# MpokiAbel/UPMEM--OpenFHE

Hardware: AMD Instinct MI355X
Metric: 64-bit coeffs/sec for NTT+Hadamard+INTT, N=2^16, 16 towers; % HBM roofline (higher is better)
Workload: dtype u64; 1 GPU; configs[2]: N=2^16, towers=16, batch=1024 per GPU, c = INTT(NTT(a) (.) b); log_n=16, towers=16, batch_per_gpu=1024, global_batch=1024, parallelism=batch-sharded x1 (no data-path collective)

## Files before the change

upmem--openfhe_amd/csrc/arith.hpp:

```cpp
#pragma once
#include <hip/hip_runtime.h>
#include <stdint.h>

namespace ofhe {

typedef uint64_t u64;
typedef uint32_t u32;

struct VgprFloor {
    __device__ __forceinline__ ~VgprFloor() { asm volatile("" ::: "v63"); }
};
#define OFHE_VGPR_FLOOR() const VgprFloor ofhe_vgpr_floor_guard_

__device__ __forceinline__ u32 lo32(u64 x) { return (u32)x; }
__device__ __forceinline__ u32 hi32(u64 x) { return (u32)(x >> 32); }
__device__ __forceinline__ u64 pack(u32 lo, u32 hi) { return ((u64)hi << 32) | lo; }

__device__ __forceinline__ u64 mad32(u32 a, u32 b, u64 c) { return (u64)a * (u64)b + c; }

__device__ __forceinline__ u64 csub(u64 x, u64 m) { return x >= m ? x - m : x; }

__device__ __noinline__ u64 umod64(u64 v, u64 m) { return v % m; }
struct SwMod {
    u64 half, nm, diff;
// ... 51 lines not shown
    }
    if (OFHE_QH_ADDC) {
        const u32 h1 = __umulhi(lo32(a), hi32(b));
        const u32 h2 = __umulhi(hi32(a), lo32(b));
        const u32 s = h1 + h2;
        return mad32(hi32(a), hi32(b), pack(s, s < h1));
    }
    const u64 m1 = mad32(lo32(a), hi32(b), 0);
    const u64 m2 = mad32(hi32(a), lo32(b), 0);
    if (OFHE_QH_MAD1) return mad32(hi32(m2), one, mad32(hi32(a), hi32(b), m1 >> 32));
    return mad32(hi32(a), hi32(b), (m1 >> 32) + (m2 >> 32));
}

__device__ __forceinline__ u64 mulhi_exact(u64 a, u64 b) {
    u64 p00 = mad32(lo32(a), lo32(b), 0);
    u64 m1 = mad32(lo32(a), hi32(b), (u64)hi32(p00));
    u64 m2 = mad32(hi32(a), lo32(b), (u64)lo32(m1));
    u64 h = mad32(hi32(a), hi32(b), (u64)hi32(m1));
    return h + (u64)hi32(m2);
}

template <bool SPQ, bool QA = false>
struct Mod {
    u64 q;
    u64 q4;
    u64 q8;
    u64 nq;
    u64 nq4;
    u64 nq8;
    u32 sh;
    u32 one = 1;
};

template <bool SPQ, bool QA>
__device__ __forceinline__ u64 shoup_lazy(u64 a, u64 w, u64 wp, const Mod<SPQ, QA>& M) {
    const u64 qh = mulhi_approx<QA>(a, wp, M.one);
    u64 s = mad32(lo32(a), lo32(w), 0);
    s = mad32(lo32(qh), lo32(M.nq), s);
    u32 hi;
    if (SPQ)
        hi = hi32(s) + lo32(a) * hi32(w) + hi32(a) * lo32(w) - (lo32(qh) << M.sh) + hi32(qh) * lo32(M.nq);
    else
        hi = hi32(s) + lo32(a) * hi32(w) + hi32(a) * lo32(w) + lo32(qh) * hi32(M.nq) + hi32(qh) * lo32(M.nq);
    return pack(lo32(s), hi);
}

// ... 120 lines not shown
```

upmem--openfhe_amd/csrc/bconv_cols.hpp:

```cpp
#pragma once
#include "bconv_mma.hpp"

namespace ofhe {

#ifndef OFHE_BCC_STAGE_BAR
#define OFHE_BCC_STAGE_BAR 1
#endif
#ifndef OFHE_BCC_MINW
#define OFHE_BCC_MINW 3
#endif
#ifndef OFHE_BCC_WAVES
#define OFHE_BCC_WAVES 12
#endif
constexpr u32 BC_WAVES = OFHE_BCC_WAVES;
constexpr u32 BC_THREADS = 64 * BC_WAVES;
constexpr u32 BC_COLS = 16, BC_ROWS = 32, BC_POS = BC_COLS * BC_ROWS;

template <bool SPQ>
__device__ __forceinline__ void bcc_icol_source(const PlanArgs& P, const BmSrc* srcc, const u64* __restrict__ xb,
                                                u32 src, u32 src_rel, u32 lane, u64* dg64) {
    constexpr u32 N = 1u << 17, COLS = N / BC_ROWS;
    const u32 col = lane & 15, qq = lane >> 4;
    const u32 ts = src_rel + src;
    const auto M = load_mod<SPQ, (bool)OFHE_QA_CI>(P.tc[ts]);
// ... 102 lines not shown
            u64 d[2];
#pragma unroll
            for (int u = 0; u < 2; u++) {
                const u32 i = 2 * pr + u;
                u64 y = 0;
                if (i < A.size_q) {
                    const BmSrc S = srcc[i];
                    y = shoup_canon(xr[k][u], S.w, S.wp, S.q);
                }
                d[u] = digits8(y);
            }
            dg[it] = i32x4{(int)lo32(d[0]), (int)hi32(d[0]), (int)lo32(d[1]), (int)hi32(d[1])};
        }
    }
    __syncthreads();
    const BmW W = bm_weights();
    const u32 c = lane & 31, h = lane >> 5, col = c & 15, par = c >> 4;
    u64* ob = out + (u64)b * A.out_stride + c0 + col;
    auto colpass = [&](u64(&vv)[16], u32 j) {
        if (j >= A.size_p) return;
        const u32 jo = j >= A.gap_at ? j + A.gap : j;
        const auto M = load_mod<SPQ, (bool)OFHE_QA_BCC>(P.tc[jo]);
        const u64* tw = P.tw + (u64)jo * N * 2;
#pragma unroll
        for (int s = 0; s < 4; s++) {
            const int hg = 8 >> s;
#pragma unroll
            for (int jb = 0; jb < (1 << s); jb++) {
                const Tw tw_ = ldtw(tw, (1u << s) + jb);
#pragma unroll
                for (int g = jb * 2 * hg; g < jb * 2 * hg + hg; g++) ct_bfly_cs(vv[g], vv[g + hg], tw_, M, (s & 1) == 0);
            }
            if (OFHE_BCC_STAGE_BAR) __builtin_amdgcn_sched_barrier(0);
        }
        u64* oj = ob + (u64)jo * N;
#pragma unroll
        for (int k = 0; k < 8; k++) {
            const u64 snd = par ? vv[k] : vv[8 + k];
            const u64 rcv = pack((u32)__shfl_xor((int)lo32(snd), 16), (u32)__shfl_xor((int)hi32(snd), 16));
            u64 xv = par ? rcv : vv[k];
            u64 yv = par ? vv[8 + k] : rcv;
            const u32 g = k + 8 * par;
            ct_bfly_cs(xv, yv, ldtw(tw, 16 + g), M, true);
            st_s(oj + (u64)(2 * g) * COLS, xv);
            st_s(oj + (u64)(2 * g + 1) * COLS, yv);
        }
    };
#pragma unroll 1
    for (u32 T = w; T < tiles; T += BC_WAVES) {
        i32x4 fa[KS];
#pragma unroll
        for (int s = 0; s < KS; s++) fa[s] = frag[(T * KS + s) * 64 + lane];
        const BmRed R0 = red[4 * T + 2 * h], R1 = red[4 * T + 2 * h + 1];
        u64 v0[16], v1[16];
        auto mma = [&](int g) {
            i32x16 acc = {};
#pragma unroll
            for (int s = 0; s < KS; s++)
                acc = __builtin_amdgcn_mfma_i32_32x32x32_i8(fa[s], dg[(2 * s + h) * BC_POS + 32 * g + c], acc, 0, 0,
                                                             0);
            return acc;
        };
        i32x16 accn = mma(0);
#pragma unroll
        for (int g = 0; g < 16; g++) {
            const i32x16 acc = accn;
// ... 19 lines not shown
```

upmem--openfhe_amd/csrc/ntt_kernels.hpp:

```cpp
#pragma once
#include "arith.hpp"

namespace ofhe {

struct TowerConst {
    u64 q;
    u64 ninv;
    u64 ninv_pre;
    u64 mu;
    u64 nq;
    u64 nq4;
    u32 nshift;
    u32 spq_sh;
    u64 qinv;
    u32 one;
    u32 pad_;
};
#ifndef OFHE_QA_TCF
#define OFHE_QA_TCF 0
#endif
#ifndef OFHE_QA_TCI
#define OFHE_QA_TCI 0
#endif
#ifndef OFHE_QA_BLK
// ... 86 lines not shown
#define OFHE_FOLD 1
#endif
#ifndef OFHE_BFLY_ACC
#define OFHE_BFLY_ACC 1
#endif
template <bool SPQ, bool QA>
__device__ __forceinline__ u64 red16(u64 x, const Mod<SPQ, QA>& M) {
    if (SPQ && OFHE_FOLD) return fold_spq(x, M);
    return csub_s(x, M.q8);
}
#ifndef OFHE_FOLD_GS
#define OFHE_FOLD_GS 0
#endif
template <bool SPQ, bool QA>
__device__ __forceinline__ u64 red8(u64 x, const Mod<SPQ, QA>& M) {
    if (SPQ && OFHE_FOLD && OFHE_FOLD_GS) return fold_spq(x, M);
    return csub_s(x, M.q4);
}
template <bool SPQ, bool QA>
__device__ __forceinline__ u64 red16_gs(u64 x, const Mod<SPQ, QA>& M) {
    if (SPQ && OFHE_FOLD && OFHE_FOLD_GS) return fold_spq(x, M);
    return csub_s(x, M.q8);
}
template <bool SPQ, bool QA>
__device__ __forceinline__ void ct_bfly_cs(u64& x, u64& y, Tw w, const Mod<SPQ, QA>& M, bool cs) {
    u64 a;
    if (OFHE_LAZY_FWD)
        a = cs ? ((SPQ && OFHE_THR) ? csub_thr8(x, M) : red16(x, M)) : x;
    else
        a = csub_s(x, M.q4);
    if (OFHE_BFLY_ACC == 2) {
        const u64 c2 = (a << 1) + M.q4;
        x = shoup_lazy_acc(y, w.w, w.wp, M, a);
        y = c2 - x;
    } else if (OFHE_BFLY_ACC) {
        x = shoup_lazy_acc(y, w.w, w.wp, M, a);
        y = (a << 1) + M.q4 - x;
    } else {
        const u64 t = shoup_lazy(y, w.w, w.wp, M);
        x = a + t;
        y = a + M.q4 - t;
    }
}
template <int CS, class M_>
__device__ __forceinline__ void ct_bfly(u64& x, u64& y, Tw w, const M_& M) {
    ct_bfly_cs(x, y, w, M, CS != 0);
// ... 41 lines not shown
    if (SPQ && OFHE_THR) x = csub_s(x, 8 * q);
    if (OFHE_LAZY_FWD) x = csub_s(x, 8 * q);
    return canon8(x, q);
}

static_assert(OFHE_LAZY_FWD, "the DIT inverse uses the alternating lazy CT butterflies");

__device__ __forceinline__ void triv_bfly(u64& x, u64& y, u64 bq) {
    const u64 s = x + y;
    y = x + bq - y;
    x = s;
}

template <int H, int CS, class M_>
__device__ __forceinline__ void dit_stage16(u64 (&v)[16], const u64* base, u32 st, const M_& M) {
    constexpr int half = 1 << H;
#pragma unroll
    for (int j = 0; j < half; j++) {
        const Tw w = ldtw(base, st * j);
#pragma unroll
        for (int g = 0; g < 16; g += 2 * half) ct_bfly<CS>(v[g + j], v[g + j + half], w, M);
    }
}
template <class M_>
__device__ __forceinline__ void dit_round16(u64 (&v)[16], const u64* dtw, u32 st, u32 r, const M_& M) {
    dit_stage16<0, 1>(v, dtw + 2 * ((u64)st + r), st, M);
    dit_stage16<1, 0>(v, dtw + 2 * ((u64)2 * st + r), st, M);
    dit_stage16<2, 1>(v, dtw + 2 * ((u64)4 * st + r), st, M);
    dit_stage16<3, 0>(v, dtw + 2 * ((u64)8 * st + r), st, M);
}

template <bool SPQ, bool QA>
__device__ __forceinline__ void dit_round3(u64 (&v)[16], const u64* dtw, const Mod<SPQ, QA>& M) {
#pragma unroll
    for (int g = 0; g < 16; g += 2) triv_bfly(v[g], v[g + 1], 2 * M.q);
#pragma unroll
    for (int g = 0; g < 16; g += 4) triv_bfly(v[g], v[g + 2], M.q4);
    {
        const Tw w = ldtw(dtw, 3);
#pragma unroll
        for (int g = 0; g < 16; g += 4) ct_bfly<0>(v[g + 1], v[g + 3], w, M);
    }
#pragma unroll
    for (int g = 0; g < 16; g += 8) triv_bfly(v[g], v[g + 4], M.q8);
#pragma unroll
    for (int j = 1; j < 4; j++) {
        const Tw w = ldtw(dtw, 4 + j);
#pragma unroll
        for (int g = 0; g < 16; g += 8) ct_bfly<0>(v[g + j], v[g + j + 4], w, M);
    }
    {
        const u64 a = red16(v[0], M), b = red16(v[8], M);
        v[0] = a;
        v[8] = b;
        triv_bfly(v[0], v[8], M.q8);
    }
#pragma unroll
    for (int j = 1; j < 8; j++) ct_bfly<1>(v[j], v[j + 8], ldtw(dtw, 8 + j), M);
}

template <bool SPQ, bool QA>
__device__ __forceinline__ u64 twist_out(u64 x, Tw f, const Mod<SPQ, QA>& M) {
    return canon4m(shoup_lazy(x, f.w, f.wp, M), M);
}

template <int S, class M_, int CS = S & 1>
__device__ __forceinline__ void fwd_stage16(u64 (&v)[16], const u64* tw, u32 M0, const M_& M) {
    constexpr int half = 8 >> S;
    const u64* base = tw + 2 * ((u64)M0 << S);
#pragma unroll
    for (int j = 0; j < (1 << S); j++) {
        Tw w = ldtw(base, j);
#pragma unroll
        for (int k = j * 2 * half; k < j * 2 * half + half; k++) ct_bfly<CS>(v[k], v[k + half], w, M);
    }
}

template <int S, class M_>
__device__ __forceinline__ void inv_stage16(u64 (&v)[16], const u64* itw, u32 M0, const M_& M) {
    constexpr int half = 8 >> S;
    const u64* base = itw + 2 * ((u64)M0 << S);
#pragma unroll
    for (int j = 0; j < (1 << S); j++) {
        Tw w = ldtw(base, j);
#pragma unroll
        for (int k = j * 2 * half; k < j * 2 * half + half; k++) gs_bfly(v[k], v[k + half], w, M);
    }
}

#ifndef OFHE_LAZY_GS
#define OFHE_LAZY_GS 1
#endif
template <class M_>
__device__ __forceinline__ void gs_bfly_b(u64& x, u64& y, Tw w, const M_& M, bool in8) {
    const u64 s = x + y;
    const u64 d = x + (in8 ? M.q8 : M.q4) - y;
    x = in8 ? red16_gs(s, M) : s;
    y = shoup_lazy(d, w.w, w.wp, M);
}
template <int S, class M_>
__device__ __forceinline__ void inv_stage16_b(u64 (&v)[16], bool (&b8)[16], const u64* itw, u32 M0, const M_& M) {
    constexpr int half = 8 >> S;
    const u64* base = itw + 2 * ((u64)M0 << S);
#pragma unroll
    for (int j = 0; j < (1 << S); j++) {
        Tw w = ldtw(base, j);
#pragma unroll
        for (int k = j * 2 * half; k < j * 2 * half + half; k++) {
            gs_bfly_b(v[k], v[k + half], w, M, b8[k] || b8[k + half]);
            b8[k] = true;
            b8[k + half] = false;
        }
    }
}
template <class M_>
__device__ __forceinline__ void inv_round16_b(u64 (&v)[16], bool (&b8)[16], const u64* itw, u32 M0, const M_& M) {
    inv_stage16_b<3>(v, b8, itw, M0, M);
    inv_stage16_b<2>(v, b8, itw, M0, M);
    inv_stage16_b<1>(v, b8, itw, M0, M);
    inv_stage16_b<0>(v, b8, itw, M0, M);
}

template <class M_>
__device__ __forceinline__ void fwd_round16(u64 (&v)[16], const u64* tw, u32 M0, const M_& M) {
    fwd_stage16<0>(v, tw, M0, M);
    fwd_stage16<1>(v, tw, M0, M);
    fwd_stage16<2>(v, tw, M0, M);
    fwd_stage16<3>(v, tw, M0, M);
}
#ifndef OFHE_FWD_CANON
#define OFHE_FWD_CANON 1
#endif
template <class M_>
__device__ __forceinline__ void fwd_round16_canon(u64 (&v)[16], const u64* tw, u32 M0, const M_& M) {
    fwd_stage16<0>(v, tw, M0, M);
    fwd_stage16<1, M_, OFHE_FWD_CANON ? 0 : 1>(v, tw, M0, M);
    fwd_stage16<2>(v, tw, M0, M);
    fwd_stage16<3>(v, tw, M0, M);
}
template <class M_>
__device__ __forceinline__ void inv_round16(u64 (&v)[16], const u64* itw, u32 M0, const M_& M) {
    inv_stage16<3>(v, itw, M0, M);
    inv_stage16<2>(v, itw, M0, M);
    inv_stage16<1>(v, itw, M0, M);
    inv_stage16<0>(v, itw, M0, M);
}

#ifndef OFHE_TW3
#define OFHE_TW3 1
#endif
#ifndef OFHE_MONT
#define OFHE_MONT 1
#endif
#ifndef OFHE_COAL
#define OFHE_COAL 1
#endif
#ifndef OFHE_COAL_B
#define OFHE_COAL_B 1
#endif
constexpr bool kMontFused = OFHE_MONT && OFHE_COAL_B;
static_assert(!(kMontFused && OFHE_THR), "Montgomery Hadamard needs the forward output < 12q");
template <int S, class M_>
__device__ __forceinline__ void fwd_stage16_t3(u64 (&v)[16], const u64* tw3, u32 U, u32 u, const M_& M) {
    constexpr int half = 8 >> S;
    const u64* base = tw3 + 2 * (u64)(((1u << S) - 1) * U);
#pragma unroll
    for (int j = 0; j < (1 << S); j++) {
        Tw w = ldtw(base + 2 * (u64)j * U, u);
#pragma unroll
        for (int k = j * 2 * half; k < j * 2 * half + half; k++) ct_bfly<S & 1>(v[k], v[k + half], w, M);
    }
}
__device__ __forceinline__ u32 lds_pad(u32 p) { return p + (p >> 4); }
constexpr u32 LDS_WORDS = 4096 + 4096 / 16;

__device__ __forceinline__ void wave_stage_in(const u64* wsrc, u64* lds, u32 tid, u64 (&out)[16]) {
    const u32 lane = tid & 63, base = (tid >> 6) * 1024;
#pragma unroll
    for (int k = 0; k < 8; k++) {
        const u64x2 v = ld2_s(wsrc + 128 * k + 2 * lane);
        const u32 p = base + 128 * k + 2 * lane;
        lds[lds_pad(p)] = v.x;
        lds[lds_pad(p) + 1] = v.y;
    }
    __builtin_amdgcn_wave_barrier();
#pragma unroll
    for (int k = 0; k < 16; k++) out[k] = lds[tid * 17 + k];
    __builtin_amdgcn_wave_barrier();
}
template <int NPRE>
__device__ __forceinline__ void wave_stage_in_pre(const u64* wsrc, u64* lds, u32 tid, const u64x2 (&pre)[NPRE > 0 ? NPRE : 1],
                                                  u64 (&out)[16]) {
    const u32 lane = tid & 63, base = (tid >> 6) * 1024;
// ... 34 lines not shown
__device__ __forceinline__ void block_body(const PlanArgs& P, const u64* src, u64* dst, const u64* __restrict__ bdat,
                                           u32 batch, u32 wid, u64* lds, u32 tid) {
    static_assert(NR == 2 || NR == 3, "k_block covers the last 8 (NR=2) or 12 (NR=3) stages");
    static_assert(SK == 0 || (SK == 3 && NR == 3), "k_block: SK = 3 needs NR = 3");
    const u32 logn = P.log_n;
    const u32 N = 1u << logn;
    const u32 G = N >> 12;
    const u32 g = wid % G;
    const u32 pb = wid / G;
    const u32 t = pb / batch, b = pb % batch;
    const u64 inner = (u64)t * N + ((u64)g << 12);
    const u64 off = (u64)b * P.dstride + inner;
    const u64 boff = (u64)b * P.bstride + inner;
    const u64* blk = src + (u64)b * P.sstride + inner;
    u64* oblk = dst + off;
    const TowerConst tc = P.tc[t];
    const u64 q = tc.q;
    const auto M = load_mod<SPQ, (bool)OFHE_QA_BLK>(tc);
    const u64* tw = P.tw + (u64)t * N * 2;
    const u32 h = tid >> 4, r = tid & 15;
    const u32 L1 = tid + h;
    const u32 L2 = h * 272 + r;
    const u32 L3 = tid * 17;
    u64 v[16];

    if (MODE == MODE_FWD || MODE == MODE_FUSED || MODE == MODE_FWD_SUB) {
        if (NR == 3) {
#pragma unroll
            for (int k = 0; k < 16; k++) v[k] = ld_s(blk + tid + 256 * k);
            if (SK == 3)
                fwd_stage16<3>(v, tw, (N >> 12) + g, M);
            else
                fwd_round16(v, tw, (N >> 12) + g, M);
#pragma unroll
            for (int k = 0; k < 16; k++) lds[L1 + 272 * k] = v[k];
            __syncthreads();
#pragma unroll
            for (int k = 0; k < 16; k++) v[k] = lds[L2 + 17 * k];
        } else {
#pragma unroll
            for (int k = 0; k < 16; k++) v[k] = ld_s(blk + h * 256 + r + 16 * k);
        }
        fwd_round16(v, tw, (N >> 8) + g * 16 + h, M);
#pragma unroll
        for (int k = 0; k < 16; k++) lds[L2 + 17 * k] = v[k];
        __syncthreads();
#pragma unroll
        for (int k = 0; k < 16; k++) v[k] = lds[L3 + k];
        constexpr int BPF = ((MODE == MODE_FUSED && OFHE_COAL_B) || MODE == MODE_FWD_SUB) ? OFHE_B_PF : 0;
        u64x2 bpre[BPF > 0 ? BPF : 1];
#pragma unroll
        for (int k = 0; k < BPF; k++) bpre[k] = ld2_s(bdat + boff + (tid >> 6) * 1024 + 128 * k + 2 * (tid & 63));
        if (OFHE_TW3) {
            const u64* tw3 = P.tw3 + (u64)t * (N / 16) * 30;
            const u32 U = N >> 4, u = g * 256 + tid;
            fwd_stage16_t3<0>(v, tw3, U, u, M);
            fwd_stage16_t3<1>(v, tw3, U, u, M);
            fwd_stage16_t3<2>(v, tw3, U, u, M);
            fwd_stage16_t3<3>(v, tw3, U, u, M);
        } else {
            fwd_round16(v, tw, (N >> 4) + g * 256 + tid, M);
        }
        if (!(MODE == MODE_FUSED && kMontFused) && MODE != MODE_FWD_SUB) {
#pragma unroll
            for (int k = 0; k < 16; k++) v[k] = canon_fwd<SPQ>(v[k], M);
        }
        if (MODE == MODE_FWD_SUB) {
            static_assert(!OFHE_THR, "the lazy forward-subtract needs the forward output < 12q (OFHE_THR widens it)");
            u64 xx[16];
            wave_stage_in_pre<BPF>(bdat + boff + (tid >> 6) * 1024, lds, tid, bpre, xx);
            const u64 sc = P.scal[3 * t + 1], scp = P.scal[3 * t + 2];
            const u64 q12 = M.q8 + M.q4;
#pragma unroll
            for (int k = 0; k < 16; k++) v[k] = canon4m(shoup_lazy(xx[k] + q12 - v[k], sc, scp, M), M);
            wave_stage_out(v, lds, tid, oblk + (tid >> 6) * 1024);
            return;
        }
        if (MODE == MODE_FWD) {
            if (OFHE_COAL) {
                wave_stage_out(v, lds, tid, oblk + (tid >> 6) * 1024);
            } else {
                ulonglong2* o = reinterpret_cast<ulonglong2*>(oblk + tid * 16);
#pragma unroll
                for (int k = 0; k < 8; k++) o[k] = make_ulonglong2(v[2 * k], v[2 * k + 1]);
// ... 23 lines not shown
                v[2 * k + 1] = barrett_ref(v[2 * k + 1], bb.y, q, tc.mu, tc.nshift);
            }
        }
    } else {
        if (OFHE_COAL) {
            wave_stage_in(blk + (tid >> 6) * 1024, lds, tid, v);
        } else {
            const ulonglong2* ip = reinterpret_cast<const ulonglong2*>(blk + tid * 16);
#pragma unroll
            for (int k = 0; k < 8; k++) {
                ulonglong2 a = ip[k];
                v[2 * k] = a.x;
                v[2 * k + 1] = a.y;
            }
        }
    }
    const u64* dtw = P.dtw + (u64)t * N * 2;
    dit_round3(v, dtw, M);
#pragma unroll
    for (int k = 0; k < 16; k++) lds[L3 + k] = v[k];
    __syncthreads();
#pragma unroll
    for (int k = 0; k < 16; k++) v[k] = lds[L2 + 17 * k];
    dit_round16(v, dtw, 16, r, M);
    const u64* tw_ = P.twist + (u64)t * N * 2 + 2 * ((u64)g << 12);
    if (NR == 2) {
#pragma unroll
        for (int k = 0; k < 16; k++) {
            const u32 p = h * 256 + r + 16 * k;
            const Tw f = ldtw(tw_, p);
            st_s(oblk + p, shoup_lazy(v[k], f.w, f.wp, M));
        }
        return;
    }
#pragma unroll
    for (int k = 0; k < 16; k++) lds[L2 + 17 * k] = v[k];
    __syncthreads();
#pragma unroll
    for (int k = 0; k < 16; k++) v[k] = lds[L1 + 272 * k];
    if (SK == 3)
        dit_stage16<0, 1>(v, dtw + 2 * ((u64)256 + tid), 256, M);
    else
        dit_round16(v, dtw, 256, tid, M);
#pragma unroll
    for (int k = 0; k < 16; k++) {
        const Tw f = ldtw(tw_, tid + 256 * k);
        v[k] = logn == 12 ? twist_out(v[k], f, M) : shoup_lazy(v[k], f.w, f.wp, M);
    }
#pragma unroll
    for (int k = 0; k < 16; k++) st_s(oblk + tid + 256 * k, v[k]);
}
template <int MODE, bool SPQ, int NR, int SK = 0>
__global__ __launch_bounds__(256, OFHE_KB_WAVES) void k_block(PlanArgs P, const u64* src, u64* dst,
                                                              const u64* __restrict__ bdat, u32 batch, u32 nwg) {
    OFHE_VGPR_FLOOR();
    __shared__ u64 lds[LDS_WORDS];
    block_body<MODE, SPQ, NR, SK>(P, src, dst, bdat, batch, xcd_remap(blockIdx.x, nwg), lds, threadIdx.x);
}

struct SwSrc {
    const u64* last;
    u64 lstride;
    u64 ql;
    const u64* tab;
    u64 pre, pre_p;
};
// ... 12 lines not shown
#ifndef OFHE_TCOLS_HALF_WAVES
#define OFHE_TCOLS_HALF_WAVES 5
#endif
constexpr u32 TCOLS_LDS_INV_WORDS = OFHE_TCOLS_HALF ? 8 * 16 * TCOLS_W : TCOLS_LDS_WORDS;
template <bool INV, bool SPQ, bool SWS = false, int LOGN = 16>
__device__ __forceinline__ void tcols_body(const PlanArgs& P, const u64* src, u64* dst, u32 batch, u32 wid,
                                           const SwSrc& SWA, u64* lds, u32 tid) {
    static_assert(LOGN == 16 || LOGN == 17, "k_tcols: N = 2^16 or 2^17");
    constexpr u32 N = 1u << LOGN, S = N / 256, W = TCOLS_W;
    const u32 cb = wid % (S / W);
    const u32 pb = wid / (S / W);
    const u32 t = pb / batch, b = pb % batch;
    const u64 inner = (u64)t * N + cb * W;
    const u64* x = src + (u64)b * P.sstride + inner;
    u64* y = dst + (u64)b * P.dstride + inner;
    const TowerConst tc = P.tc[t];
    const auto M = load_mod<SPQ, INV ? (bool)OFHE_QA_TCI : (bool)OFHE_QA_TCF>(tc);
    const u32 h = tid / W, r = tid % W;
    const u32 L1 = tid, L2 = h * 16 * W + r;
    u64 v[16];
    if (!INV) {
        const u64* tw = P.tw + (u64)t * N * 2;
        constexpr u32 RP = OFHE_TCOLS_PADF ? 16 * W + 16 : 16 * W;
        if (SWS) {
            const u64 w = SWA.tab[6 * t + 1], wp = SWA.tab[6 * t + 2];
            const SwMod sm = sw_mod(SWA.ql, tc.q);
            const u64* lp = SWA.last + (u64)b * SWA.lstride + cb * W;
#pragma unroll
            for (int k = 0; k < 16; k++) {
                u64 e = lp[(u64)(h + 16 * k) * S + r];
                if (SWA.pre != 1) e = shoup_canon(e, SWA.pre, SWA.pre_p, SWA.ql);
                e = switch_mod1(e, sm);
                v[k] = w != 1 ? shoup_canon(e, w, wp, tc.q) : e;
            }
        } else {
#pragma unroll
            for (int k = 0; k < 16; k++) v[k] = ld_s(x + (u64)(h + 16 * k) * S + r);
        }
        fwd_round16_canon(v, tw, 1, M);
#pragma unroll
        for (int k = 0; k < 16; k++) lds[L1 + RP * k] = v[k];
        __syncthreads();
#pragma unroll
        for (int k = 0; k < 16; k++) v[k] = lds[h * RP + r + W * k];
        fwd_round16(v, tw, 16 + h, M);
#pragma unroll
        for (int k = 0; k < 16; k++) st_s(y + (u64)(16 * h + k) * S + r, v[k]);
    } else {
        const u64* itw = P.itw + (u64)t * N * 2;
#pragma unroll
        for (int k = 0; k < 16; k++) v[k] = ld_s(x + (u64)(16 * h + k) * S + r);
        if (OFHE_LAZY_GS) {
            bool b8[16];
#pragma unroll
            for (int k = 0; k < 16; k++) b8[k] = false;
            inv_round16_b(v, b8, itw, 16 + h, M);
            if (OFHE_TCOLS_HALF) {
                u64 o[16];
                if (h < 8) {
#pragma unroll
                    for (int k = 0; k < 16; k++) lds[L2 + W * k] = v[k];
                }
                __syncthreads();
#pragma unroll
                for (int k = 0; k < 8; k++) o[k] = lds[L1 + 16 * W * k];
                __syncthreads();
                if (h >= 8) {
#pragma unroll
                    for (int k = 0; k < 16; k++) lds[L2 - 8 * 16 * W + W * k] = v[k];
                }
                __syncthreads();
#pragma unroll
                for (int k = 8; k < 16; k++) o[k] = lds[L1 + 16 * W * (k - 8)];
#pragma unroll
                for (int k = 0; k < 16; k++) {
                    v[k] = o[k];
                    b8[k] = true;
                }
            } else {
#pragma unroll
                for (int k = 0; k < 16; k++) lds[L2 + W * k] = v[k];
                __syncthreads();
#pragma unroll
                for (int k = 0; k < 16; k++) {
                    v[k] = lds[L1 + 16 * W * k];
                    b8[k] = true;
                }
            }
            inv_round16_b(v, b8, itw, 1, M);
#pragma unroll
            for (int k = 0; k < 16; k++)
                st_s(y + (u64)(h + 16 * k) * S + r, b8[k] ? canon8m(v[k], M) : canon4m(v[k], M));
        } else {
            inv_round16(v, itw, 16 + h, M);
#pragma unroll
            for (int k = 0; k < 16; k++) lds[L2 + W * k] = v[k];
            __syncthreads();
#pragma unroll
            for (int k = 0; k < 16; k++) v[k] = lds[L1 + 16 * W * k];
            inv_round16(v, itw, 1, M);
#pragma unroll
            for (int k = 0; k < 16; k++) st_s(y + (u64)(h + 16 * k) * S + r, canon4m(v[k], M));
        }
    }
}

template <bool INV, bool SPQ, bool SWS = false, int LOGN = 16>
__global__ __launch_bounds__(16 * TCOLS_W, (INV && OFHE_TCOLS_HALF) ? OFHE_TCOLS_HALF_WAVES : OFHE_KB_WAVES) void k_tcols(
    PlanArgs P, const u64* src, u64* dst, u32 batch, u32 nwg, SwSrc SWA) {
    OFHE_VGPR_FLOOR();
    __shared__ u64 lds[INV ? TCOLS_LDS_INV_WORDS : TCOLS_LDS_WORDS];
    tcols_body<INV, SPQ, SWS, LOGN>(P, src, dst, batch, xcd_remap(blockIdx.x, nwg), SWA, lds, threadIdx.x);
}

template <bool INV, bool SPQ>
// ... 17 lines not shown
    const u64* other = lds + (hf ^ 1) * HALF;
    const u32 L1 = tl, L2 = h * 16 * W + r;
    u64 v[16];
    if (!INV) {
        const u64* tw = P.tw + (u64)t * N * 2;
#pragma unroll
        for (int k = 0; k < 16; k++) v[k] = ld_s(x + (u64)(h + 16 * k) * S + r);
        const Tw w1 = ldtw(tw, 1);
        if (hf) {
#pragma unroll
            for (int k = 0; k < 16; k++) v[k] = shoup_lazy(v[k], w1.w, w1.wp, M);
        }
#pragma unroll
        for (int k = 0; k < 16; k++) my[L1 + 16 * W * k] = v[k];
        __syncthreads();
        if (hf) {
#pragma unroll
            for (int k = 0; k < 16; k++) v[k] = other[L1 + 16 * W * k] + M.q4 - v[k];
        } else {
#pragma unroll
            for (int k = 0; k < 16; k++) v[k] += other[L1 + 16 * W * k];
        }
        __syncthreads();
        fwd_round16(v, tw, 2 + hf, M);
#pragma unroll
        for (int k = 0; k < 16; k++) my[L1 + 16 * W * k] = v[k];
        __syncthreads();
#pragma unroll
        for (int k = 0; k < 16; k++) v[k] = my[L2 + W * k];
        fwd_round16(v, tw, 32 + 16 * hf + h, M);
#pragma unroll
        for (int k = 0; k < 16; k++) st_s(y + (u64)(16 * h + k) * S + r, v[k]);
    } else {
        const u64* itw = P.itw + (u64)t * N * 2;
#pragma unroll
        for (int k = 0; k < 16; k++) v[k] = ld_s(x + (u64)(16 * h + k) * S + r);
        inv_round16(v, itw, 32 + 16 * hf + h, M);
#pragma unroll
        for (int k = 0; k < 16; k++) my[L2 + W * k] = v[k];
        __syncthreads();
#pragma unroll
        for (int k = 0; k < 16; k++) v[k] = my[L1 + 16 * W * k];
        inv_round16(v, itw, 2 + hf, M);
#pragma unroll
        for (int k = 0; k < 16; k++) my[L1 + 16 * W * k] = v[k];
        __syncthreads();
        if (hf) {
            const Tw w1 = ldtw(itw, 1);
#pragma unroll
            for (int k = 0; k < 16; k++)
                v[k] = canon4m(shoup_lazy(other[L1 + 16 * W * k] + M.q4 - v[k], w1.w, w1.wp, M), M);
        } else {
#pragma unroll
            for (int k = 0; k < 16; k++) v[k] = canon4m(csub_s(v[k] + other[L1 + 16 * W * k], M.q4), M);
        }
#pragma unroll
        for (int k = 0; k < 16; k++) st_s(y + (u64)(h + 16 * k) * S + r, v[k]);
    }
}

template <int E, int CPT, class M_>
__device__ __forceinline__ void cols_fwd(u64 (&v)[CPT][E], const u64* tw, const M_& M) {
    constexpr int KA = __builtin_ctz(E);
#pragma unroll
    for (int s = 0; s < KA; s++) {
        const int half = E >> (s + 1);
#pragma unroll
        for (int j = 0; j < (1 << s); j++) {
            Tw w = ldtw(tw, (1u << s) + j);
#pragma unroll
            for (int k = j * 2 * half; k < j * 2 * half + half; k++)
#pragma unroll
                for (int c = 0; c < CPT; c++) ct_bfly_cs(v[c][k], v[c][k + half], w, M, ((KA - 1 - s) & 1) == 0);
        }
    }
}
template <int E, int CPT, class M_>
__device__ __forceinline__ void cols_inv(u64 (&v)[CPT][E], const u64* itw, const M_& M) {
    constexpr int KA = __builtin_ctz(E);
#pragma unroll
    for (int s = KA - 1; s >= 0; s--) {
        const int half = E >> (s + 1);
#pragma unroll
        for (int j = 0; j < (1 << s); j++) {
            Tw w = ldtw(itw, (1u << s) + j);
#pragma unroll
            for (int k = j * 2 * half; k < j * 2 * half + half; k++)
#pragma unroll
                for (int c = 0; c < CPT; c++) gs_bfly(v[c][k], v[c][k + half], w, M);
        }
    }
}
template <int E, int CPT, class M_>
__device__ __forceinline__ void cols_inv_b(u64 (&v)[CPT][E], bool (&b8)[E], const u64* itw, const M_& M) {
    constexpr int KA = __builtin_ctz(E);
#pragma unroll
    for (int k = 0; k < E; k++) b8[k] = false;
#pragma unroll
    for (int s = KA - 1; s >= 0; s--) {
        const int half = E >> (s + 1);
#pragma unroll
        for (int j = 0; j < (1 << s); j++) {
            Tw w = ldtw(itw, (1u << s) + j);
#pragma unroll
            for (int k = j * 2 * half; k < j * 2 * half + half; k++) {
                const bool in8 = b8[k] || b8[k + half];
#pragma unroll
                for (int c = 0; c < CPT; c++) gs_bfly_b(v[c][k], v[c][k + half], w, M, in8);
                b8[k] = true;
                b8[k + half] = false;
            }
        }
    }
}

template <int KA, bool INV, int CPT, bool SPQ, bool SWS = false>
__global__ __launch_bounds__(256) void k_cols(PlanArgs P, const u64* src, u64* dst, u32 batch, u32 nwg, SwSrc S) {
    OFHE_VGPR_FLOOR();
    constexpr int E = 1 << KA;
    constexpr u32 N = 1u << (KA + 12);
    constexpr u32 CB = 16 / CPT;
    const u32 wid = xcd_remap(blockIdx.x, nwg);
    const u32 cb = wid % CB;
    const u32 pb = wid / CB;
    const u32 t = pb / batch, b = pb % batch;
    const u64 inner = (u64)t * N + cb * (256 * CPT) + threadIdx.x * CPT;
    const u64* x = src + (u64)b * P.sstride + inner;
    u64* y = dst + (u64)b * P.dstride + inner;
    const TowerConst tc = P.tc[t];
    const auto M = load_mod<SPQ, INV ? (bool)OFHE_QA_CI : (bool)OFHE_QA_CF>(tc);
    u64 v[CPT][E];
    if (SWS) {
        const u64 w = S.tab[6 * t + 1], wp = S.tab[6 * t + 2];
// ... 13 lines not shown
            for (int c = 0; c < CPT; c++) {
                u64 e = lv[c];
                if (S.pre != 1) e = shoup_canon(e, S.pre, S.pre_p, S.ql);
                e = switch_mod1(e, sm);
                if (w != 1) e = shoup_canon(e, w, wp, tc.q);
                v[c][k] = e;
            }
        }
    }
#pragma unroll
    for (int k = 0; k < E && !SWS; k++) {
        if (CPT == 2) {
            const u64x2 p = ld2_s(x + (u64)k * 4096);
            v[0][k] = p.x;
            v[CPT - 1][k] = p.y;
        } else {
            v[0][k] = ld_s(x + (u64)k * 4096);
        }
    }
    if (!INV) {
        cols_fwd<E, CPT>(v, P.tw + (u64)t * N * 2, M);
    } else {
        if (OFHE_LAZY_GS) {
            bool b8[E];
            cols_inv_b<E, CPT>(v, b8, P.itw + (u64)t * N * 2, M);
#pragma unroll
            for (int k = 0; k < E; k++)
#pragma unroll
                for (int c = 0; c < CPT; c++) v[c][k] = b8[k] ? canon8m(v[c][k], M) : canon4m(v[c][k], M);
        } else {
            cols_inv<E, CPT>(v, P.itw + (u64)t * N * 2, M);
#pragma unroll
            for (int k = 0; k < E; k++)
#pragma unroll
                for (int c = 0; c < CPT; c++) v[c][k] = canon4m(v[c][k], M);
        }
    }
#pragma unroll
    for (int k = 0; k < E; k++) {
        if (CPT == 2) {
            u64x2 w;
            w.x = v[0][k];
            w.y = v[CPT - 1][k];
            st2_s(y + (u64)k * 4096, w);
        } else {
            st_s(y + (u64)k * 4096, v[0][k]);
        }
    }
}

template <int MODE, bool SPQ>
__global__ __launch_bounds__(256) void k_small(PlanArgs P, const u64* src, u64* dst, const u64* __restrict__ bdat,
// ... 56 lines not shown
```

Before: 81.68 billion coeffs/s.

## Compute lazy-reduction fold schedules at compile time from coefficient bound tracking

Adds constexpr bound tracking that searches, per NTT pass, for the minimal set of butterfly stages needing a conditional subtract or fold, instead of the fixed alternating pattern. It does the same for the inverse GS butterflies, replacing the runtime bool b8 tracking with a static per-butterfly schedule. The goal is to remove redundant modular reductions in the SPQ (special-prime) path while keeping intermediate values within the lazy bound. If any inter-kernel bound assumption is wrong, results could overflow, and static_asserts pin the expected schedules.

Measured after the change: 82.23 billion coeffs/s (median of 6 runs). No clear change (+0.7%).

```diff
diff --git a/upmem--openfhe_amd/csrc/arith.hpp b/upmem--openfhe_amd/csrc/arith.hpp
--- a/upmem--openfhe_amd/csrc/arith.hpp
+++ b/upmem--openfhe_amd/csrc/arith.hpp
@@ -97,6 +97,7 @@
 
 template <bool SPQ, bool QA = false>
 struct Mod {
+    static constexpr bool spq = SPQ;
     u64 q;
     u64 q4;
     u64 q8;
diff --git a/upmem--openfhe_amd/csrc/bconv_cols.hpp b/upmem--openfhe_amd/csrc/bconv_cols.hpp
--- a/upmem--openfhe_amd/csrc/bconv_cols.hpp
+++ b/upmem--openfhe_amd/csrc/bconv_cols.hpp
@@ -148,6 +148,8 @@
         const u32 jo = j >= A.gap_at ? j + A.gap : j;
         const auto M = load_mod<SPQ, (bool)OFHE_QA_BCC>(P.tc[jo]);
         const u64* tw = P.tw + (u64)jo * N * 2;
+        constexpr CtSched CF = LazyB<ct_tight(SPQ)>::cols_fwd(5);
+        static_assert(CF.out > 0 && CF.out <= LazyB<ct_tight(SPQ)>::block3_in, "k_bconv_cols -> k_block NR = 3");
 #pragma unroll
         for (int s = 0; s < 4; s++) {
             const int hg = 8 >> s;
@@ -155,7 +157,7 @@
             for (int jb = 0; jb < (1 << s); jb++) {
                 const Tw tw_ = ldtw(tw, (1u << s) + jb);
 #pragma unroll
-                for (int g = jb * 2 * hg; g < jb * 2 * hg + hg; g++) ct_bfly_cs(vv[g], vv[g + hg], tw_, M, (s & 1) == 0);
+                for (int g = jb * 2 * hg; g < jb * 2 * hg + hg; g++) ct_bfly_cs(vv[g], vv[g + hg], tw_, M, (CF.folds >> s) & 1);
             }
             if (OFHE_BCC_STAGE_BAR) __builtin_amdgcn_sched_barrier(0);
         }
@@ -167,7 +169,7 @@
             u64 xv = par ? rcv : vv[k];
             u64 yv = par ? vv[8 + k] : rcv;
             const u32 g = k + 8 * par;
-            ct_bfly_cs(xv, yv, ldtw(tw, 16 + g), M, true);
+            ct_bfly_cs(xv, yv, ldtw(tw, 16 + g), M, (CF.folds >> 4) & 1);
             st_s(oj + (u64)(2 * g) * COLS, xv);
             st_s(oj + (u64)(2 * g + 1) * COLS, yv);
         }
diff --git a/upmem--openfhe_amd/csrc/ntt_kernels.hpp b/upmem--openfhe_amd/csrc/ntt_kernels.hpp
--- a/upmem--openfhe_amd/csrc/ntt_kernels.hpp
+++ b/upmem--openfhe_amd/csrc/ntt_kernels.hpp
@@ -132,6 +132,94 @@
     if (SPQ && OFHE_FOLD && OFHE_FOLD_GS) return fold_spq(x, M);
     return csub_s(x, M.q8);
 }
+
+#ifndef OFHE_BOUND_SCHED
+#define OFHE_BOUND_SCHED 1
+#endif
+constexpr bool ct_tight(bool spq) { return spq && OFHE_BOUND_SCHED && OFHE_FOLD && OFHE_LAZY_FWD && !OFHE_THR; }
+#ifndef OFHE_SPQ_CANON
+#define OFHE_SPQ_CANON 1
+#endif
+constexpr bool gs_tight(bool spq) { return spq && OFHE_BOUND_SCHED >= 2 && OFHE_SPQ_CANON; }
+constexpr int kCtMaxIn = 12;
+constexpr int kLazyMax = 16;
+
+struct CtSched {
+    u32 folds;
+    int out;
+};
+constexpr int ct_run(u32 folds, int n, int in, int red) {
+    int b = in;
+    for (int s = 0; s < n; s++) {
+        if ((folds >> s) & 1) {
+            if (b > kLazyMax) return -1;
+            b = red;
+        } else if (b > kCtMaxIn) {
+            return -1;
+        }
+        b += 4;
+    }
+    return b;
+}
+constexpr CtSched ct_sched(bool tight, int n, int in, int out_max, u32 fixed) {
+    if (!tight) return CtSched{fixed, ct_run(fixed, n, in, 8)};
+    CtSched best{0, -1};
+    int bc = 99;
+    for (u32 m = 0; m < (1u << n); m++) {
+        const int c = __builtin_popcount(m);
+        if (c > bc) continue;
+        const int o = ct_run(m, n, in, 2);
+        if (o < 0 || o > out_max) continue;
+        const u32 d = m ^ best.folds;
+        if (c < bc || !(m & d & (0 - d))) {
+            best = CtSched{m, o};
+            bc = c;
+        }
+    }
+    return best;
+}
+constexpr u32 cols_fixed(int ka) {
+    u32 m = 0;
+    for (int s = 0; s < ka; s++)
+        if (((ka - 1 - s) & 1) == 0) m |= 1u << s;
+    return m;
+}
+#ifndef OFHE_FWD_CANON
+#define OFHE_FWD_CANON 1
+#endif
+template <bool T>
+struct LazyB {
+    static constexpr int fwd_in = 4;
+    static constexpr int block2_in = T ? 10 : 12;
+    static constexpr int block3_in = 12;
+    static constexpr int blocksk_in = T ? 10 : 12;
+    static constexpr int fwd_out_max = 12;
+    static constexpr int dit3_out = T ? 10 : 16;
+    static constexpr int twist_out = 4;
+    static constexpr int gs_in = 4;
+    static constexpr CtSched tcols_fwd = ct_sched(T, 8, fwd_in, block2_in, OFHE_FWD_CANON ? 0xA8 : 0xAA);
+    static constexpr CtSched tcols9_fwd = ct_sched(T, 8, fwd_in + 4, block2_in, 0xAA);
+    static constexpr CtSched block2_fwd = ct_sched(T, 8, block2_in, fwd_out_max, 0xAA);
+    static constexpr CtSched block3_fwd = ct_sched(T, 12, block3_in, fwd_out_max, 0xAAA);
+    static constexpr CtSched blocksk_fwd = ct_sched(T, 9, blocksk_in, fwd_out_max, 0x155);
+    static constexpr CtSched dit2 = ct_sched(T, 4, dit3_out, kLazyMax, 0x5);
+    static constexpr CtSched dit3 = ct_sched(T, 8, dit3_out, kLazyMax, 0x55);
+    static constexpr CtSched ditsk = ct_sched(T, 5, dit3_out, kLazyMax, 0x15);
+    static constexpr CtSched cols_fwd(int ka) { return ct_sched(T, ka, fwd_in, block3_in, cols_fixed(ka)); }
+    static_assert(tcols_fwd.out > 0 && tcols_fwd.out <= block2_in && tcols_fwd.out <= blocksk_in, "k_tcols forward -> k_block");
+    static_assert(tcols9_fwd.out > 0 && tcols9_fwd.out <= block2_in, "k_tcols9 forward -> k_block NR = 2");
+    static_assert(block2_fwd.out > 0 && block3_fwd.out > 0 && blocksk_fwd.out > 0, "k_block forward half");
+    static_assert(dit2.out > 0 && dit3.out > 0 && ditsk.out > 0, "k_block DIT rounds");
+    static_assert(twist_out <= gs_in, "k_block inverse -> inverse column pass");
+};
+static_assert(LazyB<true>::tcols_fwd.folds == 0x48 && LazyB<true>::tcols_fwd.out == 10, "N N N F | N N F N");
+static_assert(LazyB<true>::tcols9_fwd.folds == 0xA4 && LazyB<true>::tcols9_fwd.out == 6, "N N F N | N F N F");
+static_assert(LazyB<true>::block2_fwd.folds == 0x92 && LazyB<true>::block2_fwd.out == 6, "N F N N | F N N F");
+static_assert(LazyB<true>::block3_fwd.folds == 0x492 && LazyB<true>::block3_fwd.out == 10, "N F N N | F N N F | N N F N");
+static_assert(LazyB<true>::blocksk_fwd.folds == 0x92 &&LazyB<true>::blocksk_fwd.out == 10, "N | F N N F | N N F N");
+static_assert(LazyB<true>::dit2.folds == 0x2 && LazyB<true>::dit3.folds == 0x92 && LazyB<true>::ditsk.folds == 0x12, "DIT rounds");
+static_assert(LazyB<true>::cols_fwd(3).folds == 0x4 && LazyB<true>::cols_fwd(5).folds == 0x8, "k_cols forward");
+
 template <bool SPQ, bool QA>
 __device__ __forceinline__ void ct_bfly_cs(u64& x, u64& y, Tw w, const Mod<SPQ, QA>& M, bool cs) {
     u64 a;
@@ -219,12 +307,12 @@
         for (int g = 0; g < 16; g += 2 * half) ct_bfly<CS>(v[g + j], v[g + j + half], w, M);
     }
 }
-template <class M_>
+template <u32 F, class M_>
 __device__ __forceinline__ void dit_round16(u64 (&v)[16], const u64* dtw, u32 st, u32 r, const M_& M) {
-    dit_stage16<0, 1>(v, dtw + 2 * ((u64)st + r), st, M);
-    dit_stage16<1, 0>(v, dtw + 2 * ((u64)2 * st + r), st, M);
-    dit_stage16<2, 1>(v, dtw + 2 * ((u64)4 * st + r), st, M);
-    dit_stage16<3, 0>(v, dtw + 2 * ((u64)8 * st + r), st, M);
+    dit_stage16<0, F & 1>(v, dtw + 2 * ((u64)st + r), st, M);
+    dit_stage16<1, (F >> 1) & 1>(v, dtw + 2 * ((u64)2 * st + r), st, M);
+    dit_stage16<2, (F >> 2) & 1>(v, dtw + 2 * ((u64)4 * st + r), st, M);
+    dit_stage16<3, (F >> 3) & 1>(v, dtw + 2 * ((u64)8 * st + r), st, M);
 }
 
 template <bool SPQ, bool QA>
@@ -261,7 +349,7 @@
     return canon4m(shoup_lazy(x, f.w, f.wp, M), M);
 }
 
-template <int S, class M_, int CS = S & 1>
+template <int S, class M_, int CS>
 __device__ __forceinline__ void fwd_stage16(u64 (&v)[16], const u64* tw, u32 M0, const M_& M) {
     constexpr int half = 8 >> S;
     const u64* base = tw + 2 * ((u64)M0 << S);
@@ -288,52 +376,119 @@
 #ifndef OFHE_LAZY_GS
 #define OFHE_LAZY_GS 1
 #endif
+template <int E>
+struct GsSched {
+    static constexpr int KA = __builtin_ctz(E);
+    unsigned char kq[KA][E / 2];
+    unsigned char red[KA][E / 2];
+    unsigned char out[E];
+    int nred;
+};
+constexpr int gs_k(int half, int i) { return (i / half) * 2 * half + i % half; }
+constexpr int gs_i(int half, int r) { return r % (2 * half) < half ? (r / (2 * half)) * half + r % (2 * half) : -1; }
+template <int E>
+constexpr GsSched<E> gs_sched(bool tight, int red_to, int in, int out_max) {
+    GsSched<E> S{};
+    constexpr int KA = GsSched<E>::KA;
+    int b[E] = {};
+    bool bad = false;
+    for (int k = 0; k < E; k++) b[k] = in;
+    for (int si = 0; si < KA; si++) {
+        const int half = 1 << si;
+        for (int i = 0; i < E / 2; i++) {
+            const int k = gs_k(half, i), bx = b[k], by = b[k + half];
+            if (bx + by > kLazyMax) bad = true;
+            S.kq[si][i] = (unsigned char)(tight ? by : ((bx > 4 || by > 4) ? 8 : 4));
+            b[k] = bx + by;
+            b[k + half] = 4;
+        }
+        for (int i = 0; i < E / 2; i++) {
+            int r[2] = {-1, -1};
+            if (!tight) {
+                if (b[gs_k(half, i)] > 8) r[0] = gs_k(half, i);
+            } else if (si + 1 == KA) {
+                if (b[gs_k(half, i)] > out_max) r[0] = gs_k(half, i);
+            } else {
+                const int x = gs_k(2 * half, i), y = x + 2 * half;
+                const int hi = b[x] >= b[y] ? x : y, lo = x + y - hi;
+                if (b[x] + b[y] > kLazyMax) {
+                    r[0] = hi;
+                    if (red_to + b[lo] > kLazyMax) r[1] = lo;
+                }
+            }
+            for (int u = 0; u < 2; u++) {
+                if (r[u] < 0) continue;
+                const int j = gs_i(half, r[u]);
+                if (j < 0 || b[r[u]] <= red_to) {
+                    bad = true;
+                    continue;
+                }
+                S.red[si][j] = 1;
+                S.nred++;
+                b[r[u]] = red_to;
+            }
+        }
+    }
+    for (int k = 0; k < E; k++) {
+        if (b[k] > out_max) bad = true;
+        S.out[k] = (unsigned char)b[k];
+    }
+    if (bad) S.nred = -1;
+    return S;
+}
+template <int E, bool TIGHT, bool FOLD, int IN, int OUT_MAX>
+struct GsPass {
+    static constexpr GsSched<E> s = gs_sched<E>(TIGHT, (TIGHT && FOLD) ? 2 : 8, IN, OUT_MAX);
+    static_assert(s.nred >= 0, "no legal lazy GS schedule");
+};
+constexpr bool gs_fold(bool spq) { return spq && OFHE_FOLD && OFHE_FOLD_GS; }
+template <int E, bool SPQ, int IN, bool LAST>
+using GsPassOf = GsPass<E, gs_tight(SPQ), gs_fold(SPQ), IN, LAST ? (gs_tight(SPQ) ? kLazyMax : 8) : 8>;
+static_assert(GsPass<16, true, false, 4, 8>::s.nred == 12 && GsPass<16, true, false, 8, 16>::s.nred == 16 &&
+                  GsPass<16, false, false, 4, 8>::s.nred == 12 && GsPass<16, false, false, 8, 8>::s.nred == 20 &&
+                  GsPass<16, true, true, 4, 8>::s.nred == 8 && GsPass<16, true, true, 8, 16>::s.nred == 10,
+              "reductions per radix-16 GS round as documented");
+
+template <class M_>
+__device__ __forceinline__ void gs_bfly_t(u64& x, u64& y, Tw w, const M_& M, int kq, bool red) {
+    const u64 s = x + y;
+    const u64 d = x + (kq == 4 ? M.q4 : kq == 8 ? M.q8 : (u64)kq * M.q) - y;
+    x = red ? red16_gs(s, M) : s;
+    y = shoup_lazy(d, w.w, w.wp, M);
+}
 template <class M_>
 __device__ __forceinline__ void gs_bfly_b(u64& x, u64& y, Tw w, const M_& M, bool in8) {
-    const u64 s = x + y;
-    const u64 d = x + (in8 ? M.q8 : M.q4) - y;
-    x = in8 ? red16_gs(s, M) : s;
-    y = shoup_lazy(d, w.w, w.wp, M);
-}
-template <int S, class M_>
-__device__ __forceinline__ void inv_stage16_b(u64 (&v)[16], bool (&b8)[16], const u64* itw, u32 M0, const M_& M) {
-    constexpr int half = 8 >> S;
+    gs_bfly_t(x, y, w, M, in8 ? 8 : 4, in8);
+}
+template <int S, class GP, class M_>
+__device__ __forceinline__ void inv_stage16_t(u64 (&v)[16], const u64* itw, u32 M0, const M_& M) {
+    constexpr int half = 8 >> S, si = 3 - S;
+    constexpr GsSched<16> G = GP::s;
     const u64* base = itw + 2 * ((u64)M0 << S);
 #pragma unroll
     for (int j = 0; j < (1 << S); j++) {
         Tw w = ldtw(base, j);
 #pragma unroll
         for (int k = j * 2 * half; k < j * 2 * half + half; k++) {
-            gs_bfly_b(v[k], v[k + half], w, M, b8[k] || b8[k + half]);
-            b8[k] = true;
-            b8[k + half] = false;
-        }
-    }
-}
-template <class M_>
-__device__ __forceinline__ void inv_round16_b(u64 (&v)[16], bool (&b8)[16], const u64* itw, u32 M0, const M_& M) {
-    inv_stage16_b<3>(v, b8, itw, M0, M);
-    inv_stage16_b<2>(v, b8, itw, M0, M);
-    inv_stage16_b<1>(v, b8, itw, M0, M);
-    inv_stage16_b<0>(v, b8, itw, M0, M);
-}
-
-template <class M_>
+            const int i = j * half + k - j * 2 * half;
+            gs_bfly_t(v[k], v[k + half], w, M, G.kq[si][i], G.red[si][i]);
+        }
+    }
+}
+template <class GP, class M_>
+__device__ __forceinline__ void inv_round16_t(u64 (&v)[16], const u64* itw, u32 M0, const M_& M) {
+    inv_stage16_t<3, GP>(v, itw, M0, M);
+    inv_stage16_t<2, GP>(v, itw, M0, M);
+    inv_stage16_t<1, GP>(v, itw, M0, M);
+    inv_stage16_t<0, GP>(v, itw, M0, M);
+}
+
+template <u32 F, class M_>
 __device__ __forceinline__ void fwd_round16(u64 (&v)[16], const u64* tw, u32 M0, const M_& M) {
-    fwd_stage16<0>(v, tw, M0, M);
-    fwd_stage16<1>(v, tw, M0, M);
-    fwd_stage16<2>(v, tw, M0, M);
-    fwd_stage16<3>(v, tw, M0, M);
-}
-#ifndef OFHE_FWD_CANON
-#define OFHE_FWD_CANON 1
-#endif
-template <class M_>
-__device__ __forceinline__ void fwd_round16_canon(u64 (&v)[16], const u64* tw, u32 M0, const M_& M) {
-    fwd_stage16<0>(v, tw, M0, M);
-    fwd_stage16<1, M_, OFHE_FWD_CANON ? 0 : 1>(v, tw, M0, M);
-    fwd_stage16<2>(v, tw, M0, M);
-    fwd_stage16<3>(v, tw, M0, M);
+    fwd_stage16<0, M_, F & 1>(v, tw, M0, M);
+    fwd_stage16<1, M_, (F >> 1) & 1>(v, tw, M0, M);
+    fwd_stage16<2, M_, (F >> 2) & 1>(v, tw, M0, M);
+    fwd_stage16<3, M_, (F >> 3) & 1>(v, tw, M0, M);
 }
 template <class M_>
 __device__ __forceinline__ void inv_round16(u64 (&v)[16], const u64* itw, u32 M0, const M_& M) {
@@ -357,7 +512,7 @@
 #endif
 constexpr bool kMontFused = OFHE_MONT && OFHE_COAL_B;
 static_assert(!(kMontFused && OFHE_THR), "Montgomery Hadamard needs the forward output < 12q");
-template <int S, class M_>
+template <int S, int CS, class M_>
 __device__ __forceinline__ void fwd_stage16_t3(u64 (&v)[16], const u64* tw3, u32 U, u32 u, const M_& M) {
     constexpr int half = 8 >> S;
     const u64* base = tw3 + 2 * (u64)(((1u << S) - 1) * U);
@@ -365,7 +520,7 @@
     for (int j = 0; j < (1 << S); j++) {
         Tw w = ldtw(base + 2 * (u64)j * U, u);
 #pragma unroll
-        for (int k = j * 2 * half; k < j * 2 * half + half; k++) ct_bfly<S & 1>(v[k], v[k + half], w, M);
+        for (int k = j * 2 * half; k < j * 2 * half + half; k++) ct_bfly<CS>(v[k], v[k + half], w, M);
     }
 }
 __device__ __forceinline__ u32 lds_pad(u32 p) { return p + (p >> 4); }
@@ -446,6 +601,11 @@
     const u32 L1 = tid + h;
     const u32 L2 = h * 272 + r;
     const u32 L3 = tid * 17;
+    using LB = LazyB<ct_tight(SPQ)>;
+    constexpr CtSched FS = SK == 3 ? LB::blocksk_fwd : NR == 3 ? LB::block3_fwd : LB::block2_fwd;
+    constexpr CtSched DS = SK == 3 ? LB::ditsk : NR == 3 ? LB::dit3 : LB::dit2;
+    constexpr int FO = SK == 3 ? 1 : NR == 3 ? 4 : 0;
+    static_assert(FS.out <= LB::fwd_out_max, "mont_mul and the forward-subtract need the forward output < 12q");
     u64 v[16];
 
     if (MODE == MODE_FWD || MODE == MODE_FUSED || MODE == MODE_FWD_SUB) {
@@ -453,9 +613,9 @@
 #pragma unroll
             for (int k = 0; k < 16; k++) v[k] = ld_s(blk + tid + 256 * k);
             if (SK == 3)
-                fwd_stage16<3>(v, tw, (N >> 12) + g, M);
+                fwd_stage16<3, Mod<SPQ, (bool)OFHE_QA_BLK>, FS.folds & 1>(v, tw, (N >> 12) + g, M);
             else
-                fwd_round16(v, tw, (N >> 12) + g, M);
+                fwd_round16<FS.folds & 15>(v, tw, (N >> 12) + g, M);
 #pragma unroll
             for (int k = 0; k < 16; k++) lds[L1 + 272 * k] = v[k];
             __syncthreads();
@@ -465,7 +625,7 @@
 #pragma unroll
             for (int k = 0; k < 16; k++) v[k] = ld_s(blk + h * 256 + r + 16 * k);
         }
-        fwd_round16(v, tw, (N >> 8) + g * 16 + h, M);
+        fwd_round16<(FS.folds >> FO) & 15>(v, tw, (N >> 8) + g * 16 + h, M);
 #pragma unroll
         for (int k = 0; k < 16; k++) lds[L2 + 17 * k] = v[k];
         __syncthreads();
@@ -478,12 +638,13 @@
         if (OFHE_TW3) {
             const u64* tw3 = P.tw3 + (u64)t * (N / 16) * 30;
             const u32 U = N >> 4, u = g * 256 + tid;
-            fwd_stage16_t3<0>(v, tw3, U, u, M);
-            fwd_stage16_t3<1>(v, tw3, U, u, M);
-            fwd_stage16_t3<2>(v, tw3, U, u, M);
-            fwd_stage16_t3<3>(v, tw3, U, u, M);
+            constexpr u32 F3 = FS.folds >> (FO + 4);
+            fwd_stage16_t3<0, F3 & 1>(v, tw3, U, u, M);
+            fwd_stage16_t3<1, (F3 >> 1) & 1>(v, tw3, U, u, M);
+            fwd_stage16_t3<2, (F3 >> 2) & 1>(v, tw3, U, u, M);
+            fwd_stage16_t3<3, (F3 >> 3) & 1>(v, tw3, U, u, M);
         } else {
-            fwd_round16(v, tw, (N >> 4) + g * 256 + tid, M);
+            fwd_round16<(FS.folds >> (FO + 4)) & 15>(v, tw, (N >> 4) + g * 256 + tid, M);
         }
         if (!(MODE == MODE_FUSED && kMontFused) && MODE != MODE_FWD_SUB) {
 #pragma unroll
@@ -553,7 +714,7 @@
     __syncthreads();
 #pragma unroll
     for (int k = 0; k < 16; k++) v[k] = lds[L2 + 17 * k];
-    dit_round16(v, dtw, 16, r, M);
+    dit_round16<DS.folds & 15>(v, dtw, 16, r, M);
     const u64* tw_ = P.twist + (u64)t * N * 2 + 2 * ((u64)g << 12);
     if (NR == 2) {
 #pragma unroll
@@ -570,9 +731,9 @@
 #pragma unroll
     for (int k = 0; k < 16; k++) v[k] = lds[L1 + 272 * k];
     if (SK == 3)
-        dit_stage16<0, 1>(v, dtw + 2 * ((u64)256 + tid), 256, M);
+        dit_stage16<0, (DS.folds >> 4) & 1>(v, dtw + 2 * ((u64)256 + tid), 256, M);
     else
-        dit_round16(v, dtw, 256, tid, M);
+        dit_round16<(DS.folds >> 4) & 15>(v, dtw, 256, tid, M);
 #pragma unroll
     for (int k = 0; k < 16; k++) {
         const Tw f = ldtw(tw_, tid + 256 * k);
@@ -631,6 +792,7 @@
     if (!INV) {
         const u64* tw = P.tw + (u64)t * N * 2;
         constexpr u32 RP = OFHE_TCOLS_PADF ? 16 * W + 16 : 16 * W;
+        constexpr CtSched TF = LazyB<ct_tight(SPQ)>::tcols_fwd;
         if (SWS) {
             const u64 w = SWA.tab[6 * t + 1], wp = SWA.tab[6 * t + 2];
             const SwMod sm = sw_mod(SWA.ql, tc.q);
@@ -646,13 +808,13 @@
 #pragma unroll
             for (int k = 0; k < 16; k++) v[k] = ld_s(x + (u64)(h + 16 * k) * S + r);
         }
-        fwd_round16_canon(v, tw, 1, M);
+        fwd_round16<TF.folds & 15>(v, tw, 1, M);
 #pragma unroll
         for (int k = 0; k < 16; k++) lds[L1 + RP * k] = v[k];
         __syncthreads();
 #pragma unroll
         for (int k = 0; k < 16; k++) v[k] = lds[h * RP + r + W * k];
-        fwd_round16(v, tw, 16 + h, M);
+        fwd_round16<(TF.folds >> 4) & 15>(v, tw, 16 + h, M);
 #pragma unroll
         for (int k = 0; k < 16; k++) st_s(y + (u64)(16 * h + k) * S + r, v[k]);
     } else {
@@ -660,10 +822,9 @@
 #pragma unroll
         for (int k = 0; k < 16; k++) v[k] = ld_s(x + (u64)(16 * h + k) * S + r);
         if (OFHE_LAZY_GS) {
-            bool b8[16];
-#pragma unroll
-            for (int k = 0; k < 16; k++) b8[k] = false;
-            inv_round16_b(v, b8, itw, 16 + h, M);
+            using G1 = GsPassOf<16, SPQ, LazyB<false>::gs_in, false>;
+            using G2 = GsPassOf<16, SPQ, 8, true>;
+            inv_round16_t<G1>(v, itw, 16 + h, M);
             if (OFHE_TCOLS_HALF) {
                 u64 o[16];
                 if (h < 8) {
@@ -682,24 +843,19 @@
 #pragma unroll
                 for (int k = 8; k < 16; k++) o[k] = lds[L1 + 16 * W * (k - 8)];
 #pragma unroll
-                for (int k = 0; k < 16; k++) {
-                    v[k] = o[k];
-                    b8[k] = true;
-                }
+                for (int k = 0; k < 16; k++) v[k] = o[k];
             } else {
 #pragma unroll
                 for (int k = 0; k < 16; k++) lds[L2 + W * k] = v[k];
                 __syncthreads();
 #pragma unroll
-                for (int k = 0; k < 16; k++) {
-                    v[k] = lds[L1 + 16 * W * k];
-                    b8[k] = true;
-                }
+                for (int k = 0; k < 16; k++) v[k] = lds[L1 + 16 * W * k];
             }
-            inv_round16_b(v, b8, itw, 1, M);
+            inv_round16_t<G2>(v, itw, 1, M);
+            constexpr GsSched<16> GO = G2::s;
 #pragma unroll
             for (int k = 0; k < 16; k++)
-                st_s(y + (u64)(h + 16 * k) * S + r, b8[k] ? canon8m(v[k], M) : canon4m(v[k], M));
+                st_s(y + (u64)(h + 16 * k) * S + r, GO.out[k] > 4 ? canon8m(v[k], M) : canon4m(v[k], M));
         } else {
             inv_round16(v, itw, 16 + h, M);
 #pragma unroll
@@ -763,13 +919,14 @@
             for (int k = 0; k < 16; k++) v[k] += other[L1 + 16 * W * k];
         }
         __syncthreads();
-        fwd_round16(v, tw, 2 + hf, M);
+        constexpr CtSched TF = LazyB<ct_tight(SPQ)>::tcols9_fwd;
+        fwd_round16<TF.folds & 15>(v, tw, 2 + hf, M);
 #pragma unroll
         for (int k = 0; k < 16; k++) my[L1 + 16 * W * k] = v[k];
         __syncthreads();
 #pragma unroll
         for (int k = 0; k < 16; k++) v[k] = my[L2 + W * k];
-        fwd_round16(v, tw, 32 + 16 * hf + h, M);
+        fwd_round16<(TF.folds >> 4) & 15>(v, tw, 32 + 16 * hf + h, M);
 #pragma unroll
         for (int k = 0; k < 16; k++) st_s(y + (u64)(16 * h + k) * S + r, v[k]);
     } else {
@@ -803,6 +960,8 @@
 template <int E, int CPT, class M_>
 __device__ __forceinline__ void cols_fwd(u64 (&v)[CPT][E], const u64* tw, const M_& M) {
     constexpr int KA = __builtin_ctz(E);
+    constexpr CtSched CF = LazyB<ct_tight(M_::spq)>::cols_fwd(KA);
+    static_assert(CF.out > 0 && CF.out <= LazyB<ct_tight(M_::spq)>::block3_in, "k_cols forward -> k_block NR = 3");
 #pragma unroll
     for (int s = 0; s < KA; s++) {
         const int half = E >> (s + 1);
@@ -812,7 +971,7 @@
 #pragma unroll
             for (int k = j * 2 * half; k < j * 2 * half + half; k++)
 #pragma unroll
-                for (int c = 0; c < CPT; c++) ct_bfly_cs(v[c][k], v[c][k + half], w, M, ((KA - 1 - s) & 1) == 0);
+                for (int c = 0; c < CPT; c++) ct_bfly_cs(v[c][k], v[c][k + half], w, M, (CF.folds >> s) & 1);
         }
     }
 }
@@ -832,11 +991,10 @@
         }
     }
 }
-template <int E, int CPT, class M_>
-__device__ __forceinline__ void cols_inv_b(u64 (&v)[CPT][E], bool (&b8)[E], const u64* itw, const M_& M) {
+template <int E, int CPT, class GP, class M_>
+__device__ __forceinline__ void cols_inv_t(u64 (&v)[CPT][E], const u64* itw, const M_& M) {
     constexpr int KA = __builtin_ctz(E);
-#pragma unroll
-    for (int k = 0; k < E; k++) b8[k] = false;
+    constexpr GsSched<E> G = GP::s;
 #pragma unroll
     for (int s = KA - 1; s >= 0; s--) {
         const int half = E >> (s + 1);
@@ -845,11 +1003,9 @@
             Tw w = ldtw(itw, (1u << s) + j);
 #pragma unroll
             for (int k = j * 2 * half; k < j * 2 * half + half; k++) {
-                const bool in8 = b8[k] || b8[k + half];
-#pragma unroll
-                for (int c = 0; c < CPT; c++) gs_bfly_b(v[c][k], v[c][k + half], w, M, in8);
-                b8[k] = true;
-                b8[k + half] = false;
+                const int si = KA - 1 - s, i = j * half + k - j * 2 * half;
+#pragma unroll
+                for (int c = 0; c < CPT; c++) gs_bfly_t(v[c][k], v[c][k + half], w, M, G.kq[si][i], G.red[si][i]);
             }
         }
     }
@@ -909,12 +1065,13 @@
         cols_fwd<E, CPT>(v, P.tw + (u64)t * N * 2, M);
     } else {
         if (OFHE_LAZY_GS) {
-            bool b8[E];
-            cols_inv_b<E, CPT>(v, b8, P.itw + (u64)t * N * 2, M);
+            using GP = GsPassOf<E, SPQ, LazyB<false>::gs_in, true>;
+            cols_inv_t<E, CPT, GP>(v, P.itw + (u64)t * N * 2, M);
+            constexpr GsSched<E> GO = GP::s;
 #pragma unroll
             for (int k = 0; k < E; k++)
 #pragma unroll
-                for (int c = 0; c < CPT; c++) v[c][k] = b8[k] ? canon8m(v[c][k], M) : canon4m(v[c][k], M);
+                for (int c = 0; c < CPT; c++) v[c][k] = GO.out[k] > 4 ? canon8m(v[c][k], M) : canon4m(v[c][k], M);
         } else {
             cols_inv<E, CPT>(v, P.itw + (u64)t * N * 2, M);
 #pragma unroll
```
